# hits-mbm-dev/grappa

Hardware: AMD Instinct MI355X
Metric: molecules/sec (train step, energy+force loss) (higher is better)
Workload: dtype f32

## Files before the change

grappa_amd/_lib.py:

```python
import ctypes as C
import os

from . import settings

_HERE = os.path.dirname(os.path.abspath(__file__))
LIB_PATH = settings.read("LIB_PATH") or os.path.join(_HERE, "libgrappa_hip.so")

ABI_VERSION = 11
GEMM_GROUP4_MAX = 4
GEMM_GROUP_MAX = 16
GEMM_PRECISIONS = {"f32": 0, "f32_bf16x9": 1, "f32_bf16x6": 2, "bf16x3": 3, "bf16": 4, "f32_f16x3": 5}

c_float_p = C.POINTER(C.c_float)
c_int_p = C.POINTER(C.c_int)


class GemmDesc(C.Structure):
    _fields_ = [("M", C.c_int), ("N", C.c_int), ("K", C.c_int), ("a_kcontig", C.c_int), ("b_kcontig", C.c_int),
                ("A", C.c_void_p), ("lda", C.c_int), ("B", C.c_void_p), ("ldb", C.c_int), ("C", C.c_void_p), ("ldc", C.c_int),
                ("C2", C.c_void_p), ("ldc2", C.c_int), ("bias", C.c_void_p), ("res", C.c_void_p), ("ldres", C.c_int),
                ("aux", C.c_void_p), ("ldaux", C.c_int), ("pre", C.c_void_p), ("ldpre", C.c_int), ("a_colsum", C.c_void_p), ("act", C.c_int), ("drop_p", C.c_float), ("drop_seed", C.c_uint64),
                ("accumulate", C.c_int), ("precision", C.c_int),
                ("a_planes", C.c_int), ("b_planes", C.c_int), ("a_plane_stride", C.c_size_t), ("b_plane_stride", C.c_size_t),
                ("Cp", C.c_void_p), ("ldcp", C.c_int), ("cp_plane_stride", C.c_size_t),
                ("resp", C.c_void_p), ("ldresp", C.c_int), ("resp_plane_stride", C.c_size_t),
                ("auxp", C.c_void_p), ("ldauxp", C.c_int), ("auxp_plane_stride", C.c_size_t),
                ("cp_nplanes", C.c_int), ("resp_nplanes", C.c_int), ("auxp_nplanes", C.c_int), ("C1p", C.c_void_p), ("ldc1p", C.c_int),
                ("a_amax", C.c_void_p), ("b_amax", C.c_void_p), ("amax_bcast", C.c_int), ("out_amax", C.c_void_p),
                ("res_ln_mean", C.c_void_p), ("res_ln_rstd", C.c_void_p), ("res_ln_gamma", C.c_void_p), ("res_ln_beta", C.c_void_p),
                ("a_rowmax", C.c_void_p), ("b_rowmax", C.c_void_p),
                ("out_amax_parts", C.c_void_p), ("a_amax_nseg", C.c_int),
                ("plan_cfg", C.c_int), ("plan_nsplit", C.c_int), ("plan_tail", C.c_int), ("splitk_reduce", C.c_int), ("drop_salt", C.c_void_p)]


class LnFwdItem(C.Structure):
    _fields_ = [("M", C.c_int), ("W", C.c_int), ("x", C.c_void_p), ("ldx", C.c_int), ("gamma", C.c_void_p), ("beta", C.c_void_p), ("y", C.c_void_p),
                ("ldy", C.c_int), ("mean", C.c_void_p), ("rstd", C.c_void_p), ("y_amax", C.c_void_p)]


class LnBwdItem(C.Structure):
    _fields_ = [("M", C.c_int), ("W", C.c_int), ("dy", C.c_void_p), ("lddy", C.c_int), ("x", C.c_void_p), ("ldx", C.c_int), ("mean", C.c_void_p),
                ("rstd", C.c_void_p), ("gamma", C.c_void_p), ("dx", C.c_void_p), ("lddx", C.c_int), ("part", C.c_void_p), ("dx_amax", C.c_void_p)]


class ActDropoutItem(C.Structure):
    _fields_ = [("M", C.c_int), ("N", C.c_int), ("dy", C.c_void_p), ("lddy", C.c_int), ("y", C.c_void_p), ("ldy", C.c_int), ("drop_p", C.c_float),
                ("drop_seed", C.c_uint64), ("dz", C.c_void_p), ("lddz", C.c_int), ("dz_amax", C.c_void_p), ("drop_salt", C.c_void_p)]
# ... 97 lines not shown
    "grappa_split_planes_f32": (_i, [_vp, _i, _i, _vp, _i, _vp, _i, _sz, _i]),
    "grappa_split_pairs_f32": (_i, [_vp, _i, _i, _vp, _i, _vp, _vp, _i, _i]),
    "grappa_split_pairs_f32_batched": (_i, [_vp, _i, _i, _vp]),
    "grappa_amax_f32_workspace_bytes": (_sz, [_i, _i]),
    "grappa_amax_f32": (_i, [_vp, _i, _i, _vp, _i, _vp, _vp, _vp, _sz]),
    "grappa_amax_f32_batched": (_i, [_vp, _i, _vp]),
    "grappa_amax_reduce": (_i, [_vp, _i, C.POINTER(C.c_void_p), C.POINTER(C.c_int), _vp]),
    "grappa_amax_combine": (_i, [_vp, _i, _i, _vp, _vp]),
    "grappa_gemm_f32_workspace_bytes": (_sz, [_i, _i, _i]),
    "grappa_gemm_f32_plan": (_i, [_i, _i, _i, _i, c_int_p, c_int_p, c_int_p, c_int_p, c_int_p]),
    "grappa_gemm_f32_plan_desc": (_i, [C.POINTER(GemmDesc), c_int_p, c_int_p, c_int_p, c_int_p, c_int_p]),
    "grappa_gemm_f32_workspace_bytes_desc": (_sz, [C.POINTER(GemmDesc)]),
    "grappa_gemm_f32": (_i, [_vp, C.POINTER(GemmDesc), _vp, _sz]),
    "grappa_gemm_f32_grouped_workspace_bytes": (_sz, [C.POINTER(GemmDesc), _i]),
    "grappa_gemm_f32_grouped": (_i, [_vp, C.POINTER(GemmDesc), _i, _vp, _sz]),
    "grappa_gemm_f32_group_workspace_bytes": (_sz, [C.POINTER(GemmDesc), _i]),
    "grappa_gemm_f32_group": (_i, [_vp, C.POINTER(GemmDesc), _i, _vp, _sz]),
    "grappa_colsum_workspace_bytes": (_sz, [_i, _i]),
    "grappa_colsum_f32": (_i, [_vp, _i, _i, _vp, _i, _vp, _i, _vp, _sz]),
    "grappa_act_dropout_bwd_f32": (_i, [_vp, _i, _i, _vp, _i, _vp, _i, _f, _u64, _vp, _i, _vp]),
    "grappa_act_dropout_bwd_amax_f32": (_i, [_vp, _i, _i, _vp, _i, _vp, _i, _f, _u64, _vp, _i, _vp, _vp]),
    "grappa_layernorm_fwd_batched_f32": (_i, [_vp, C.POINTER(LnFwdItem), _i]),
    "grappa_layernorm_bwd_batched_f32": (_i, [_vp, C.POINTER(LnBwdItem), _i]),
    "grappa_act_dropout_bwd_batched_f32": (_i, [_vp, C.POINTER(ActDropoutItem), _i]),
    "grappa_seqattn_fwd_batched_f32": (_i, [_vp, C.POINTER(SeqAttnItem), _i]),
    "grappa_seqattn_bwd_batched_f32": (_i, [_vp, C.POINTER(SeqAttnItem), _i]),
    "grappa_act_dropout_bwd_pairs_f32": (_i, [_vp, _i, _i, _vp, _i, _vp, _i, _f, _u64, _vp, _i, _vp, _vp, _i, _vp]),
    "grappa_add_f32": (_i, [_vp, _sz, _vp, _vp, _vp]),
    "grappa_layernorm_fwd_f32": (_i, [_vp, _i, _i, _vp, _i, _vp, _vp, _vp, _i, _vp, _vp]),
    "grappa_layernorm_fwd_pairs_f32": (_i, [_vp, _i, _i, _vp, _i, _vp, _vp, _vp, _i, _vp, _vp, _vp, _vp, _i]),
# ... 134 lines not shown
```

grappa_amd/csrc/gemm_bf16x.hip:

```cpp
#include "gemm_common.h"

using namespace grappa_gemm;

#define GRAPPA_DECL(NAME)                                                                   \
    int grappa_bf16x_launch_##NAME(hipStream_t st, GemmParams& p, bool vec_kcontig);        \
    int grappa_bf16x_launch_group4_##NAME(hipStream_t st, const GemmGroup4& g, bool b_kcontig); \
    int grappa_bf16x_launch_grouped_##NAME(hipStream_t st, const GemmParams* d_ps, const int* d_wg_begin, int nprob, int total_wgs, bool vec, int psrc)
GRAPPA_DECL(x9);
GRAPPA_DECL(x6);
GRAPPA_DECL(x3);
GRAPPA_DECL(x1);
GRAPPA_DECL(h3);
#undef GRAPPA_DECL

int grappa_launch_gemm_bf16x_grouped(hipStream_t st, const GemmParams* d_ps, const int* d_wg_begin, int nprob, int total_wgs, int precision, bool vec, int psrc) {
    switch (precision) {
        case GRAPPA_GEMM_F32_BF16X9: return grappa_bf16x_launch_grouped_x9(st, d_ps, d_wg_begin, nprob, total_wgs, vec, psrc);
        case GRAPPA_GEMM_F32_BF16X6: return grappa_bf16x_launch_grouped_x6(st, d_ps, d_wg_begin, nprob, total_wgs, vec, psrc);
        case GRAPPA_GEMM_BF16X3: return grappa_bf16x_launch_grouped_x3(st, d_ps, d_wg_begin, nprob, total_wgs, vec, psrc);
        case GRAPPA_GEMM_BF16: return grappa_bf16x_launch_grouped_x1(st, d_ps, d_wg_begin, nprob, total_wgs, vec, psrc);
        case GRAPPA_GEMM_F32_F16X3: return grappa_bf16x_launch_grouped_h3(st, d_ps, d_wg_begin, nprob, total_wgs, vec, psrc);
        default: return GRAPPA_ERR_ARG;
    }
}

int grappa_launch_gemm_bf16x(hipStream_t st, GemmParams& p, int precision, bool vec_kcontig) {
    switch (precision) {
        case GRAPPA_GEMM_F32_BF16X9: return grappa_bf16x_launch_x9(st, p, vec_kcontig);
        case GRAPPA_GEMM_F32_BF16X6: return grappa_bf16x_launch_x6(st, p, vec_kcontig);
        case GRAPPA_GEMM_BF16X3: return grappa_bf16x_launch_x3(st, p, vec_kcontig);
        case GRAPPA_GEMM_BF16: return grappa_bf16x_launch_x1(st, p, vec_kcontig);
        case GRAPPA_GEMM_F32_F16X3: return grappa_bf16x_launch_h3(st, p, vec_kcontig);
        default: return GRAPPA_ERR_ARG;
    }
}

// ... 12 lines not shown
```

grappa_amd/csrc/gemm_bf16x_impl.h:

```cpp
#include "gemm_common.h"

using namespace grappa_gemm;

#ifndef GB_KNOCK
#define GB_KNOCK 0
#endif
#ifndef GB_STAGGER
#define GB_STAGGER 0
#endif

typedef __bf16 bf16x8 __attribute__((ext_vector_type(8)));
typedef __bf16 bf16x2 __attribute__((ext_vector_type(2)));
typedef _Float16 f16x8 __attribute__((ext_vector_type(8)));
typedef _Float16 f16x2 __attribute__((ext_vector_type(2)));

namespace {

constexpr int SK = 16;
constexpr int ROWB = 48;
#ifndef GB_AHEAD
#define GB_AHEAD 4
#endif
constexpr int AHEAD = GB_AHEAD;

// ... 327 lines not shown
    }
    __builtin_amdgcn_sched_barrier(0);
    if (!(GB_KNOCK == 5 && !TAIL)) __syncthreads();
    __builtin_amdgcn_sched_barrier(0);
    if (do_store && !(GB_KNOCK == 4 && !TAIL)) read_frags<NP, BM, BN, TM, TN, AV, BV>(nxt, wm0, wn0, lane, fn);
    if (GB_KNOCK == 4 && !TAIL) fn = fc;
    mfma_range<MODE, TM, TN, NFIRST, NM>(fc, acc);
    if (!TAIL) {
        __builtin_amdgcn_sched_group_barrier(0x002, 4, 0);
        ReadOrder<0, NM - NFIRST, (TM + TN) * NP + (AV ? TM * NP : 0) + (BV ? TN * NP : 0)>::emit();
    }
    __builtin_amdgcn_sched_barrier(0);
}

template <int NT, int MODE, int BM, int BN, int WN, bool AK, bool BKC, bool VEC, bool KMV, int PSRC = 0>
__device__ __forceinline__ void gemm_bf16x_body(const GemmParams& p, int nwg, int wgid) {
    static_assert(PSRC == 0 || (MODE == H3 && KMV && !AK && !BKC), "pair-format sources: the wgrad layout of the fp16-split arithmetic only");
    static_assert(PSRC >= 0 && PSRC <= 3, "PSRC 4 (formats per product) is resolved by the grouped kernel");
    constexpr bool pa_ = (PSRC & 1) != 0, pb_ = (PSRC & 2) != 0;
    constexpr int NP = Pieces<MODE>::NP, TM = 2, TN = BN / WN / 32;
    constexpr int NQA = BM * 4 / NT, NQB = BN * 4 / NT;
    constexpr bool AV = !AK && KMV, BV = !BKC && KMV;
    constexpr int PA = PieceBytes<BM, AV>::value;
    static_assert((NT / 64 / WN) * 64 == BM, "wavefront grid must cover the tile");
    extern __shared__ char smem[];
    const grappa_gemm_desc& d = p.d;
    if (GB_STAGGER > 0 && wgid < 256) {
        const int ph = (wgid >> 3) & 3;
        for (int i = 0; i < ph; ++i) __builtin_amdgcn_s_sleep(GB_STAGGER);
    }
    const TileCoord tc = map_logical(p, nwg, wgid);
    const int split = tc.split, tile_local = tc.tile_local, tile_n = tc.tile_n;
    const int m0 = tc.tile_m * BM, n0 = tile_n * BN;
    const int wave = threadIdx.x >> 6, lane = threadIdx.x & 63;
    const int wm0 = (wave / WN) * 64, wn0 = (wave % WN) * (BN / WN);
    const int lr = lane & 31, lh = lane >> 5;
    KRange kr;
    kr.kbeg = split * p.k_per_split;
    kr.kend = min(d.K, kr.kbeg + p.k_per_split);
    kr.nsteps = (kr.kend - kr.kbeg + SK - 1) / SK;
    const int nsteps = kr.nsteps;

    f32x16 acc[TM][TN];
#pragma unroll
    for (int i = 0; i < TM; ++i)
#pragma unroll
// ... 119 lines not shown
                for (int e = 0; e < 16; ++e) t += acc[i][j][e];
        if (t == 123.456f) p.d.C[0] = t;
        return;
    }
    tile_epilogue_rows<BM, BN, TM, TN>(p, acc, reinterpret_cast<float*>(smem + wave * EPI_WAVE_BYTES), m0, n0, wm0, wn0, lane, split, tile_local,
                                       p.vec_io != 0);
    if (p.nsplit > 1 && p.tickets) splitk_finish_tile<NT>(p, tile_local, reinterpret_cast<volatile int*>(smem));
}

template <int NT, int MODE, int BM, int BN, int WN, bool AK, bool BKC, bool VEC, bool KMV>
__global__ __launch_bounds__(NT, 2) void gemm_bf16x_kernel(GemmParams p) {
    gemm_bf16x_body<NT, MODE, BM, BN, WN, AK, BKC, VEC, KMV>(p, gridDim.x, blockIdx.x);
}

template <int NT, int MODE, int BM, int BN, int WN, bool AK, bool BKC, bool VEC, bool KMV, int PSRC = 0>
__global__ __launch_bounds__(NT, 2) void gemm_bf16x_grouped_kernel(const GemmParams* __restrict__ ps, const int* __restrict__ wg_begin, int nprob) {
    const int wg = blockIdx.x;
    int g = 0;
    while (g + 1 < nprob && wg >= wg_begin[g + 1]) ++g;
    if constexpr (PSRC == 4) {
        const int f = (ps[g].d.a_planes ? 1 : 0) | (ps[g].d.b_planes ? 2 : 0);
        const int nwg = wg_begin[g + 1] - wg_begin[g], id = wg - wg_begin[g];
        if (f == 0) gemm_bf16x_body<NT, MODE, BM, BN, WN, AK, BKC, VEC, KMV, 0>(ps[g], nwg, id);
        else if (f == 1) gemm_bf16x_body<NT, MODE, BM, BN, WN, AK, BKC, VEC, KMV, 1>(ps[g], nwg, id);
        else if (f == 2) gemm_bf16x_body<NT, MODE, BM, BN, WN, AK, BKC, VEC, KMV, 2>(ps[g], nwg, id);
        else gemm_bf16x_body<NT, MODE, BM, BN, WN, AK, BKC, VEC, KMV, 3>(ps[g], nwg, id);
    } else {
        gemm_bf16x_body<NT, MODE, BM, BN, WN, AK, BKC, VEC, KMV, PSRC>(ps[g], wg_begin[g + 1] - wg_begin[g], wg - wg_begin[g]);
    }
}

template <int NT, int MODE, int BM, int BN, int WN, bool AK, bool BKC, bool VEC, bool KMV>
__global__ __launch_bounds__(NT, 2) void gemm_bf16x_group4_kernel(GemmGroup4 g) {
    const int i = group4_find(g, blockIdx.x);
    gemm_bf16x_body<NT, MODE, BM, BN, WN, AK, BKC, VEC, KMV>(g.p[i], g.wg_begin[i + 1] - g.wg_begin[i], blockIdx.x - g.wg_begin[i]);
}

template <int NT, int MODE, int BM, int BN, int WN, bool AK, bool BKC, bool VEC, bool KMV>
int launch_group4_mode(hipStream_t st, const GemmGroup4& g) {
    constexpr size_t stages = 2 * (size_t)Pieces<MODE>::NP * (PieceBytes<BM, !AK && KMV>::value + PieceBytes<BN, !BKC && KMV>::value);
    constexpr size_t staging = (NT / 64) * (size_t)EPI_WAVE_BYTES;
    constexpr size_t smem = stages > staging ? stages : staging;
    auto kern = gemm_bf16x_group4_kernel<NT, MODE, BM, BN, WN, AK, BKC, VEC, KMV>;
// ... 27 lines not shown
int launch_layout(hipStream_t st, GemmParams& p, bool vec) {
    const grappa_gemm_desc& d = p.d;
    if (d.a_kcontig && d.b_kcontig) return vec ? launch_mode<NT, MODE, BM, BN, WN, true, true, true, false>(st, p) : launch_mode<NT, MODE, BM, BN, WN, true, true, false, false>(st, p);
    if (d.a_kcontig) return vec ? launch_mode<NT, MODE, BM, BN, WN, true, false, true, true>(st, p) : launch_mode<NT, MODE, BM, BN, WN, true, false, false, false>(st, p);
    return vec ? launch_mode<NT, MODE, BM, BN, WN, false, false, false, true>(st, p) : launch_mode<NT, MODE, BM, BN, WN, false, false, false, false>(st, p);
}

template <int MODE>
int launch_tile(hipStream_t st, GemmParams& p, bool vec) {
    if (p.bm == 256 && p.bn == 128) return launch_layout<512, MODE, 256, 128, 2>(st, p, vec);
    if (p.bm == 128 && p.bn == 128) return launch_layout<512, MODE, 128, 128, 4>(st, p, vec);
    return GRAPPA_ERR_ARG;
}

template <int MODE, bool KMV, int PSRC = 0>
int launch_grouped_wgrad(hipStream_t st, const GemmParams* d_ps, const int* d_wg_begin, int nprob, int total_wgs) {
    constexpr int NT = 512, BM = 256, BN = 128;
    constexpr size_t stages = 2 * (size_t)Pieces<MODE>::NP * (PieceBytes<BM, KMV>::value + PieceBytes<BN, KMV>::value);
    constexpr size_t staging = (NT / 64) * (size_t)EPI_WAVE_BYTES;
    constexpr size_t smem = stages > staging ? stages : staging;
    auto kern = gemm_bf16x_grouped_kernel<NT, MODE, BM, BN, 2, false, false, false, KMV, PSRC>;
    static bool attr_set = false;
    if (!attr_set) {
        if (hipFuncSetAttribute(reinterpret_cast<const void*>(kern), hipFuncAttributeMaxDynamicSharedMemorySize, (int)smem) != hipSuccess)
            return GRAPPA_ERR_LAUNCH;
        attr_set = true;
    }
    GRAPPA_LAUNCH(kern, dim3(total_wgs), dim3(NT), smem, st, d_ps, d_wg_begin, nprob);
    return grappa_launch_status();
}

}

template <int MODE>
int launch_group4(hipStream_t st, const GemmGroup4& g, bool b_kcontig) {
    if (b_kcontig) return launch_group4_mode<512, MODE, 256, 128, 2, true, true, true, false>(st, g);
    return launch_group4_mode<512, MODE, 256, 128, 2, true, false, true, true>(st, g);
}

#define GRAPPA_BF16X_MODE_FUNCS(MODE, NAME)                                                                                                  \
    int grappa_bf16x_launch_##NAME(hipStream_t st, GemmParams& p, bool vec_kcontig) { return launch_tile<MODE>(st, p, vec_kcontig); }       \
    int grappa_bf16x_launch_group4_##NAME(hipStream_t st, const GemmGroup4& g, bool b_kcontig) { return launch_group4<MODE>(st, g, b_kcontig); } \
    int grappa_bf16x_launch_grouped_##NAME(hipStream_t st, const GemmParams* d_ps, const int* d_wg_begin, int nprob, int total_wgs, bool vec, \
                                           int psrc) {                                                                                     \
        if constexpr (MODE == H3) {                                                                                                        \
            if (psrc != 0 && !vec) return GRAPPA_ERR_ARG;                                                                                  \
            if (psrc == 1) return launch_grouped_wgrad<MODE, true, 1>(st, d_ps, d_wg_begin, nprob, total_wgs);                             \
            if (psrc == 2) return launch_grouped_wgrad<MODE, true, 2>(st, d_ps, d_wg_begin, nprob, total_wgs);                             \
            if (psrc == 3) return launch_grouped_wgrad<MODE, true, 3>(st, d_ps, d_wg_begin, nprob, total_wgs);                             \
            if (psrc == 4) return launch_grouped_wgrad<MODE, true, 4>(st, d_ps, d_wg_begin, nprob, total_wgs);                             \
        } else if (psrc != 0) {                                                                                                            \
            return GRAPPA_ERR_ARG;                                                                                                         \
        }                                                                                                                                  \
        return vec ? launch_grouped_wgrad<MODE, true>(st, d_ps, d_wg_begin, nprob, total_wgs)                                              \
                   : launch_grouped_wgrad<MODE, false>(st, d_ps, d_wg_begin, nprob, total_wgs);                                            \
    }
```

grappa_amd/csrc/gemm_common.h:

```cpp
#pragma once
#include "common.h"

#ifndef GRAPPA_EPI_RES_LN
#define GRAPPA_EPI_RES_LN 1
#endif

typedef float f32x16 __attribute__((ext_vector_type(16)));

#ifndef GB_KNOCK
#define GB_KNOCK 0
#endif
namespace grappa_gemm {

constexpr int GEMM_BK = 32;

struct GemmParams {
    grappa_gemm_desc d;
    int k_per_split;
    int nsplit;
    float* slab;
    float* cs_slab;
    float drop_scale;
    int tiles_m, tiles_n;
    int tile_begin;
// ... 118 lines not shown
struct TileCoord {
    int split, tile_local, tile_m, tile_n;
};
__device__ inline TileCoord map_logical(const GemmParams& p, int nwg, int orig) {
    const int xcd = orig & 7, q = nwg >> 3, r = nwg & 7;
    const int wgid = (xcd < r ? xcd * (q + 1) : r * (q + 1) + (xcd - r) * q) + (orig >> 3);
    TileCoord t;
    t.split = wgid / p.ntiles_launch;
    t.tile_local = wgid - t.split * p.ntiles_launch;
    const int tile = p.tile_begin + t.tile_local;
    t.tile_m = tile / p.tiles_n;
    t.tile_n = tile % p.tiles_n;
    return t;
}
__device__ inline TileCoord map_workgroup(const GemmParams& p) { return map_logical(p, gridDim.x, blockIdx.x); }

template <int BM, int BN, int TM, int TN>
__device__ inline void tile_epilogue(const GemmParams& p, const f32x16 (&acc)[TM][TN], int m0, int n0, int wm0, int wn0, int lr, int lh,
                                     int split, int tile_local) {
    const grappa_gemm_desc& d = p.d;
    int ncol[TN];
    float bcol[TN];
#pragma unroll
    for (int j = 0; j < TN; ++j) {
        ncol[j] = n0 + wn0 + j * 32 + lr;
        bcol[j] = (d.bias && ncol[j] < d.N) ? d.bias[ncol[j]] : 0.0f;
    }
#pragma unroll
    for (int i = 0; i < TM; ++i)
#pragma unroll
// ... 361 lines not shown
```

grappa_amd/csrc/gemm_f32.hip:

```cpp
#include <cstdlib>
#include "gemm_common.h"

using namespace grappa_gemm;

int grappa_launch_gemm_bf16x(hipStream_t st, GemmParams& p, int precision, bool vec_kcontig);
int grappa_launch_gemm_planes(hipStream_t st, GemmParams& p, int precision);
int grappa_launch_gemm_pairs(hipStream_t st, GemmParams& p);
int grappa_launch_amax_combine(hipStream_t st, int M, int nseg, const unsigned* part, unsigned* out);
int grappa_launch_gemm_bf16x_group4(hipStream_t st, const GemmGroup4& g, int precision, bool b_kcontig);
int grappa_launch_gemm_pairs_group4(hipStream_t st, const GemmGroup4& g);
int grappa_launch_amax_combine4(hipStream_t st, int count, const int* M, const int* nseg, const unsigned* const* part, unsigned* const* out);
int grappa_launch_gemm_bf16x_grouped(hipStream_t st, const GemmParams* d_ps, const int* d_wg_begin, int nprob, int total_wgs, int precision, bool vec, int psrc);

namespace {

constexpr int BK = GEMM_BK;
constexpr int NTHREADS = 256;


template <int BROW, bool KCONT>
struct Tile {
    static constexpr int SIZE = KCONT ? BROW * (BK + 1) : BK * BROW;
    static constexpr int NV = BROW * BK / 4 / NTHREADS;
};

template <int BROW, bool KCONT>
__device__ inline void load_tile_vec(const float* __restrict__ src, int ld, int row0, int k0, int R, int Kend,
// ... 496 lines not shown
}

namespace {
constexpr int GROUP_MAX = GRAPPA_GEMM_GROUP_MAX;
struct GroupUpload {
    GemmParams p[8];
};
struct GroupIndex {
    int wg_begin[GROUP_MAX + 1], blk_begin[GROUP_MAX + 1];
};
__global__ void group_upload_kernel(GroupUpload u, int n, GemmParams* dst) {
    const int words = (int)(sizeof(GemmParams) / 4);
    for (int i = threadIdx.x; i < n * words; i += blockDim.x)
        reinterpret_cast<unsigned*>(dst)[i] = reinterpret_cast<const unsigned*>(u.p)[i];
}
__global__ void group_index_kernel(GroupIndex ix, int n, int* dst_wg, int* dst_blk, int* tickets, int ntickets) {
    for (int i = threadIdx.x; i <= n; i += blockDim.x) {
        dst_wg[i] = ix.wg_begin[i];
        dst_blk[i] = ix.blk_begin[i];
    }
    for (int i = threadIdx.x; i < ntickets; i += blockDim.x) tickets[i] = 0;
}

struct GroupPlan {
    int kps;
    int nsplit[GROUP_MAX], tiles[GROUP_MAX];
    int total_wgs;
    size_t slab_floats[GROUP_MAX], cs_floats[GROUP_MAX];
    size_t header_bytes, ticket_offset, total_bytes;
    int total_tickets;
};

bool pair_operand_ok(const void* q, int ld, int rows, const uint32_t* rowmax, int precision, int bcast_bit, int amax_bcast) {
    return precision == GRAPPA_GEMM_F32_F16X3 && rowmax != nullptr && (amax_bcast & bcast_bit) != 0 && (reinterpret_cast<uintptr_t>(q) & 15) == 0 &&
           (ld & 7) == 0 && (rows & 31) == 0 && ld >= 2 * rows;
// ... 37 lines not shown
        const double cost = (double)((wgs + 255) / 256) * 32768.0 * (kps + 160.0) / 307.0 + slab;
        if (cost < best) {
            best = cost;
            g.kps = kps;
        }
    }
    g.total_wgs = 0;
    size_t off = 0;
    for (int i = 0; i < n; ++i) {
        g.nsplit[i] = (descs[i].K + g.kps - 1) / g.kps;
        g.total_wgs += g.tiles[i] * g.nsplit[i];
        g.slab_floats[i] = g.nsplit[i] > 1 ? (size_t)g.nsplit[i] * g.tiles[i] * 256 * 128 : 0;
        g.cs_floats[i] = g.nsplit[i] > 1 ? (size_t)g.nsplit[i] * descs[i].M : 0;
        off += g.slab_floats[i] + g.cs_floats[i];
    }
    g.header_bytes = ((size_t)n * sizeof(GemmParams) + 2 * (GROUP_MAX + 1) * sizeof(int) + 255) / 256 * 256;
    g.ticket_offset = g.header_bytes + off * sizeof(float);
    g.total_tickets = 0;
    for (int i = 0; i < n; ++i) g.total_tickets += g.nsplit[i] > 1 ? g.tiles[i] : 0;
    g.total_bytes = g.ticket_offset + (size_t)g.total_tickets * sizeof(int);
    return g;
}
}

extern "C" size_t grappa_gemm_f32_grouped_workspace_bytes(const grappa_gemm_desc* descs, int n) {
    if (!descs || n <= 0 || n > GROUP_MAX) return 0;
    return plan_group(descs, n).total_bytes;
}

extern "C" int grappa_gemm_f32_grouped(void* stream, const grappa_gemm_desc* descs, int n, void* ws, size_t ws_bytes) {
    if (!descs || n <= 0 || n > GROUP_MAX) return GRAPPA_ERR_ARG;
    const int precision = descs[0].precision;
    int psrc = (descs[0].a_planes ? 1 : 0) | (descs[0].b_planes ? 2 : 0);
    for (int i = 0; i < n; ++i) {
        if (!group_desc_ok(descs[i], precision)) return GRAPPA_ERR_ARG;
        if (((descs[i].a_planes ? 1 : 0) | (descs[i].b_planes ? 2 : 0)) != psrc) psrc = 4;
    }
    const GroupPlan g = plan_group(descs, n);
    if (!ws || ws_bytes < g.total_bytes) return GRAPPA_ERR_WORKSPACE;
    hipStream_t st = reinterpret_cast<hipStream_t>(stream);
    GemmParams* d_ps = reinterpret_cast<GemmParams*>(ws);
    int* d_wg = reinterpret_cast<int*>(reinterpret_cast<char*>(ws) + (size_t)n * sizeof(GemmParams));
    int* d_blk = d_wg + (GROUP_MAX + 1);
    float* slab = reinterpret_cast<float*>(reinterpret_cast<char*>(ws) + g.header_bytes);
    GroupIndex ix;
    GroupUpload up;
    ix.wg_begin[0] = ix.blk_begin[0] = 0;
    const bool in_kernel = splitk_in_kernel(descs[0]);
    int* tickets = reinterpret_cast<int*>(reinterpret_cast<char*>(ws) + g.ticket_offset);
    int* next_ticket = tickets;
    auto al16 = [](const void* q, int ld) { return q == nullptr || ((reinterpret_cast<uintptr_t>(q) & 15) == 0 && (ld & 3) == 0); };
    int total_blocks = 0;
    bool vec = true;
    for (int i = 0; i < n; ++i) {
        const grappa_gemm_desc& d = descs[i];
        vec = vec && (reinterpret_cast<uintptr_t>(d.A) & 15) == 0 && (d.lda & 3) == 0 && ((d.M + 3) & ~3) <= d.lda &&
              (reinterpret_cast<uintptr_t>(d.B) & 15) == 0 && (d.ldb & 3) == 0 && ((d.N + 3) & ~3) <= d.ldb;
    }
// ... 26 lines not shown
            p.vec_io = al16(d.C, d.ldc) && al16(d.C2, d.ldc2) && al16(d.pre, d.ldpre) && al16(d.res, d.ldres) && al16(d.aux, d.ldaux);
            p.amax_part = nullptr;
            p.amax_seg = 32;
            p.epi_class = 0;
            ix.wg_begin[i + 1] = ix.wg_begin[i] + g.tiles[i] * g.nsplit[i];
            int blocks = 0;
            if (p.nsplit > 1 && !in_kernel) {
                blocks = (int)(((size_t)g.tiles[i] * 256 * 128 / 4 + REDUCE_THREADS - 1) / REDUCE_THREADS);
                if (blocks > 1024) blocks = 1024;
            }
            ix.blk_begin[i + 1] = ix.blk_begin[i] + blocks;
            total_blocks = ix.blk_begin[i + 1];
        }
        GRAPPA_LAUNCH(group_upload_kernel, dim3(1), dim3(256), 0, st, up, cnt, d_ps + i0);
    }
    GRAPPA_LAUNCH(group_index_kernel, dim3(1), dim3(256), 0, st, ix, n, d_wg, d_blk, tickets, in_kernel ? g.total_tickets : 0);
    if (grappa_launch_status() != GRAPPA_OK) return GRAPPA_ERR_LAUNCH;
    int rc = grappa_launch_gemm_bf16x_grouped(st, d_ps, d_wg, n, g.total_wgs, precision, vec, psrc);
    if (rc != GRAPPA_OK) return rc;
    if (total_blocks > 0) {
        GRAPPA_LAUNCH(gemm_splitk_reduce_grouped_kernel, dim3(total_blocks), dim3(REDUCE_THREADS), 0, st, d_ps, d_blk, n);
        rc = grappa_launch_status();
    }
    return rc;
}

extern "C" int grappa_gemm_f32(void* stream, const grappa_gemm_desc* d, void* ws, size_t ws_bytes) {
    if (!d || !d->A || !d->B || (!d->C && !d->Cp && !d->C1p)) return GRAPPA_ERR_ARG;
    if (!d->C && (d->C2 || d->accumulate)) return GRAPPA_ERR_ARG;
    if (d->C1p && (d->C || d->C2) ) return GRAPPA_ERR_ARG;
    if (d->C1p && !d->Cp) return GRAPPA_ERR_ARG;
    for (int np : {d->cp_nplanes, d->resp_nplanes, d->auxp_nplanes})
        if (np != 0 && np != 1 && np != 3) return GRAPPA_ERR_ARG;
// ... 220 lines not shown
```

include/grappa_hip.h:

```cpp
#ifndef GRAPPA_HIP_H
#define GRAPPA_HIP_H

#include <stddef.h>
#include <stdint.h>

#ifdef __cplusplus
extern "C" {
#endif

#define GRAPPA_OK 0
#define GRAPPA_ERR_ARG (-1)
#define GRAPPA_ERR_LAUNCH (-2)
#define GRAPPA_ERR_WORKSPACE (-3)

#define GRAPPA_ABI_VERSION 11
int grappa_abi_version(void);
const char* grappa_build_arch(void);
long long grappa_launch_count(int reset);

#define GRAPPA_ACT_NONE 0
#define GRAPPA_ACT_ELU 1

#define GRAPPA_GEMM_F32_MFMA 0
#define GRAPPA_GEMM_F32_BF16X9 1
// ... 19 lines not shown
    uint64_t drop_seed;
    int accumulate;
    int precision;
    int a_planes, b_planes;
    size_t a_plane_stride, b_plane_stride;
    uint16_t* Cp; int ldcp; size_t cp_plane_stride;
    const uint16_t* resp; int ldresp; size_t resp_plane_stride;
    const uint16_t* auxp; int ldauxp; size_t auxp_plane_stride;
    int cp_nplanes, resp_nplanes, auxp_nplanes;
    uint16_t* C1p; int ldc1p;
    const uint32_t* a_amax; const uint32_t* b_amax; int amax_bcast;
    uint32_t* out_amax;
    const float* res_ln_mean; const float* res_ln_rstd; const float* res_ln_gamma; const float* res_ln_beta;
    const uint32_t* a_rowmax; const uint32_t* b_rowmax;
    uint32_t* out_amax_parts; int a_amax_nseg;
    int plan_cfg, plan_nsplit, plan_tail, splitk_reduce;
    const uint64_t* drop_salt;
} grappa_gemm_desc;

size_t grappa_amax_f32_workspace_bytes(int R, int C);
int grappa_amax_f32(void* stream, int R, int C, const float* x, int ldx, uint32_t* row_amax, uint32_t* col_amax, void* ws, size_t ws_bytes);
typedef struct grappa_amax_item {
    const float* x; int R, C, ld, pad_;
    uint32_t* row_amax; uint32_t* col_amax;
} grappa_amax_item;
int grappa_amax_f32_batched(void* stream, int count, const grappa_amax_item* descs);
int grappa_amax_reduce(void* stream, int count, const uint32_t* const* in, const int* n, uint32_t* out);
int grappa_amax_combine(void* stream, int M, int nseg, const uint32_t* parts, uint32_t* out);

int grappa_split_planes_f32(void* stream, int R, int C, const float* x, int ldx, uint16_t* planes, int ldp, size_t plane_stride,
                            int transpose);
// ... 2 lines not shown
typedef struct grappa_split_pairs_item {
    const float* x; const uint32_t* amax; uint16_t* pairs;
    int R, C, ldx, ldp, transpose, tile_begin;
} grappa_split_pairs_item;
int grappa_split_pairs_f32_batched(void* stream, int count, int total_tiles, const grappa_split_pairs_item* items);

size_t grappa_gemm_f32_workspace_bytes(int M, int N, int K);
size_t grappa_gemm_f32_workspace_bytes_desc(const grappa_gemm_desc* d);
int grappa_gemm_f32_plan(int M, int N, int K, int precision, int* tile_m, int* tile_n, int* nsplit, int* tail_tiles, int* tail_nsplit);
int grappa_gemm_f32_plan_desc(const grappa_gemm_desc* d, int* tile_m, int* tile_n, int* nsplit, int* tail_tiles, int* tail_nsplit);
int grappa_gemm_f32(void* stream, const grappa_gemm_desc* d, void* ws, size_t ws_bytes);

#define GRAPPA_GEMM_GROUP_MAX 16
size_t grappa_gemm_f32_grouped_workspace_bytes(const grappa_gemm_desc* descs, int n);
int grappa_gemm_f32_grouped(void* stream, const grappa_gemm_desc* descs, int n, void* ws, size_t ws_bytes);
size_t grappa_gemm_f32_group_workspace_bytes(const grappa_gemm_desc* descs, int n);
int grappa_gemm_f32_group(void* stream, const grappa_gemm_desc* descs, int n, void* ws, size_t ws_bytes);

size_t grappa_colsum_workspace_bytes(int M, int N);
int grappa_colsum_f32(void* stream, int M, int N, const float* x, int ldx, float* out, int accumulate,
                      void* ws, size_t ws_bytes);

int grappa_act_dropout_bwd_f32(void* stream, int M, int N, const float* dy, int lddy, const float* y, int ldy,
                               float drop_p, uint64_t drop_seed, float* dz, int lddz, const uint64_t* drop_salt);
int grappa_act_dropout_bwd_amax_f32(void* stream, int M, int N, const float* dy, int lddy, const float* y, int ldy,
                                    float drop_p, uint64_t drop_seed, float* dz, int lddz, uint32_t* dz_amax, const uint64_t* drop_salt);
#define GRAPPA_ROW_BATCH_MAX 4
typedef struct grappa_ln_fwd_item {
    int M, W; const float* x; int ldx; const float* gamma; const float* beta; float* y; int ldy; float* mean; float* rstd; uint32_t* y_amax;
} grappa_ln_fwd_item;
// ... 340 lines not shown
```

Measured before the change: 7735.

## Deal grouped wgrad GEMM split-K slices across eight queues by cost

Adds a host-side scheduler that breaks each grouped wgrad GEMM problem into per-split slices, sorts them by cost (tiles times K range), and greedily assigns them to eight queues interleaved by workgroup id (wg&7). The assignment packs slices into 32-tile chunks and is uploaded as a GroupSlices table. The grouped kernel then maps each workgroup straight to (problem, split, tile) instead of walking wg_begin in linear order. The goal is to balance long and short K slices across XCD-like queues and cut tail imbalance. In exchange it enlarges the workspace header, may launch padding workgroups that exit early, and adds host work on every call.

Result: no change. 7768, median of 6 (+0.4%).

```diff
diff --git a/grappa_amd/_lib.py b/grappa_amd/_lib.py
--- a/grappa_amd/_lib.py
+++ b/grappa_amd/_lib.py
@@ -30,7 +30,9 @@
                 ("res_ln_mean", C.c_void_p), ("res_ln_rstd", C.c_void_p), ("res_ln_gamma", C.c_void_p), ("res_ln_beta", C.c_void_p),
                 ("a_rowmax", C.c_void_p), ("b_rowmax", C.c_void_p),
                 ("out_amax_parts", C.c_void_p), ("a_amax_nseg", C.c_int),
-                ("plan_cfg", C.c_int), ("plan_nsplit", C.c_int), ("plan_tail", C.c_int), ("splitk_reduce", C.c_int), ("drop_salt", C.c_void_p)]
+                ("plan_cfg", C.c_int), ("plan_nsplit", C.c_int), ("plan_tail", C.c_int), ("splitk_reduce", C.c_int),
+                ("wgrad_order", C.c_int),
+                ("drop_salt", C.c_void_p)]
 
 
 class LnFwdItem(C.Structure):
@@ -158,6 +160,7 @@
     "grappa_gemm_f32": (_i, [_vp, C.POINTER(GemmDesc), _vp, _sz]),
     "grappa_gemm_f32_grouped_workspace_bytes": (_sz, [C.POINTER(GemmDesc), _i]),
     "grappa_gemm_f32_grouped": (_i, [_vp, C.POINTER(GemmDesc), _i, _vp, _sz]),
+    "grappa_gemm_f32_grouped_order": (_i, [C.POINTER(GemmDesc), _i, c_int_p, _i]),
     "grappa_gemm_f32_group_workspace_bytes": (_sz, [C.POINTER(GemmDesc), _i]),
     "grappa_gemm_f32_group": (_i, [_vp, C.POINTER(GemmDesc), _i, _vp, _sz]),
     "grappa_colsum_workspace_bytes": (_sz, [_i, _i]),
diff --git a/grappa_amd/csrc/gemm_bf16x.hip b/grappa_amd/csrc/gemm_bf16x.hip
--- a/grappa_amd/csrc/gemm_bf16x.hip
+++ b/grappa_amd/csrc/gemm_bf16x.hip
@@ -5,7 +5,7 @@
 #define GRAPPA_DECL(NAME)                                                                   \
     int grappa_bf16x_launch_##NAME(hipStream_t st, GemmParams& p, bool vec_kcontig);        \
     int grappa_bf16x_launch_group4_##NAME(hipStream_t st, const GemmGroup4& g, bool b_kcontig); \
-    int grappa_bf16x_launch_grouped_##NAME(hipStream_t st, const GemmParams* d_ps, const int* d_wg_begin, int nprob, int total_wgs, bool vec, int psrc)
+    int grappa_bf16x_launch_grouped_##NAME(hipStream_t st, const GemmParams* d_ps, const int* d_wg_begin, int nprob, int total_wgs, bool vec, int psrc, const GroupSlices* d_slices)
 GRAPPA_DECL(x9);
 GRAPPA_DECL(x6);
 GRAPPA_DECL(x3);
@@ -13,13 +13,13 @@
 GRAPPA_DECL(h3);
 #undef GRAPPA_DECL
 
-int grappa_launch_gemm_bf16x_grouped(hipStream_t st, const GemmParams* d_ps, const int* d_wg_begin, int nprob, int total_wgs, int precision, bool vec, int psrc) {
+int grappa_launch_gemm_bf16x_grouped(hipStream_t st, const GemmParams* d_ps, const int* d_wg_begin, int nprob, int total_wgs, int precision, bool vec, int psrc, const GroupSlices* d_slices) {
     switch (precision) {
-        case GRAPPA_GEMM_F32_BF16X9: return grappa_bf16x_launch_grouped_x9(st, d_ps, d_wg_begin, nprob, total_wgs, vec, psrc);
-        case GRAPPA_GEMM_F32_BF16X6: return grappa_bf16x_launch_grouped_x6(st, d_ps, d_wg_begin, nprob, total_wgs, vec, psrc);
-        case GRAPPA_GEMM_BF16X3: return grappa_bf16x_launch_grouped_x3(st, d_ps, d_wg_begin, nprob, total_wgs, vec, psrc);
-        case GRAPPA_GEMM_BF16: return grappa_bf16x_launch_grouped_x1(st, d_ps, d_wg_begin, nprob, total_wgs, vec, psrc);
-        case GRAPPA_GEMM_F32_F16X3: return grappa_bf16x_launch_grouped_h3(st, d_ps, d_wg_begin, nprob, total_wgs, vec, psrc);
+        case GRAPPA_GEMM_F32_BF16X9: return grappa_bf16x_launch_grouped_x9(st, d_ps, d_wg_begin, nprob, total_wgs, vec, psrc, d_slices);
+        case GRAPPA_GEMM_F32_BF16X6: return grappa_bf16x_launch_grouped_x6(st, d_ps, d_wg_begin, nprob, total_wgs, vec, psrc, d_slices);
+        case GRAPPA_GEMM_BF16X3: return grappa_bf16x_launch_grouped_x3(st, d_ps, d_wg_begin, nprob, total_wgs, vec, psrc, d_slices);
+        case GRAPPA_GEMM_BF16: return grappa_bf16x_launch_grouped_x1(st, d_ps, d_wg_begin, nprob, total_wgs, vec, psrc, d_slices);
+        case GRAPPA_GEMM_F32_F16X3: return grappa_bf16x_launch_grouped_h3(st, d_ps, d_wg_begin, nprob, total_wgs, vec, psrc, d_slices);
         default: return GRAPPA_ERR_ARG;
     }
 }
diff --git a/grappa_amd/csrc/gemm_bf16x_impl.h b/grappa_amd/csrc/gemm_bf16x_impl.h
--- a/grappa_amd/csrc/gemm_bf16x_impl.h
+++ b/grappa_amd/csrc/gemm_bf16x_impl.h
@@ -365,7 +365,7 @@
 }
 
 template <int NT, int MODE, int BM, int BN, int WN, bool AK, bool BKC, bool VEC, bool KMV, int PSRC = 0>
-__device__ __forceinline__ void gemm_bf16x_body(const GemmParams& p, int nwg, int wgid) {
+__device__ __forceinline__ void gemm_bf16x_body(const GemmParams& p, int nwg, int wgid, const TileCoord* given = nullptr) {
     static_assert(PSRC == 0 || (MODE == H3 && KMV && !AK && !BKC), "pair-format sources: the wgrad layout of the fp16-split arithmetic only");
     static_assert(PSRC >= 0 && PSRC <= 3, "PSRC 4 (formats per product) is resolved by the grouped kernel");
     constexpr bool pa_ = (PSRC & 1) != 0, pb_ = (PSRC & 2) != 0;
@@ -380,7 +380,7 @@
         const int ph = (wgid >> 3) & 3;
         for (int i = 0; i < ph; ++i) __builtin_amdgcn_s_sleep(GB_STAGGER);
     }
-    const TileCoord tc = map_logical(p, nwg, wgid);
+    const TileCoord tc = given ? *given : map_logical(p, nwg, wgid);
     const int split = tc.split, tile_local = tc.tile_local, tile_n = tc.tile_n;
     const int m0 = tc.tile_m * BM, n0 = tile_n * BN;
     const int wave = threadIdx.x >> 6, lane = threadIdx.x & 63;
@@ -530,19 +530,34 @@
 }
 
 template <int NT, int MODE, int BM, int BN, int WN, bool AK, bool BKC, bool VEC, bool KMV, int PSRC = 0>
-__global__ __launch_bounds__(NT, 2) void gemm_bf16x_grouped_kernel(const GemmParams* __restrict__ ps, const int* __restrict__ wg_begin, int nprob) {
+__global__ __launch_bounds__(NT, 2) void gemm_bf16x_grouped_kernel(const GemmParams* __restrict__ ps, const int* __restrict__ wg_begin, int nprob,
+                                                                   const GroupSlices* __restrict__ slices) {
     const int wg = blockIdx.x;
-    int g = 0;
-    while (g + 1 < nprob && wg >= wg_begin[g + 1]) ++g;
+    int g = 0, nwg = 0, id = 0;
+    TileCoord tc;
+    if (slices) {
+        const int q = wg & 7, e = wg >> 3;
+        if (e >= slices->qend[q]) return;
+        int i = slices->qbeg[q];
+        const int last = slices->qbeg[q + 1] - 1;
+        while (i < last && e >= slices->tile0[i + 1]) ++i;
+        const int sl = slices->slice[i];
+        g = sl & 15;
+        tc = map_given(ps[g], sl >> 4, e - slices->tile0[i]);
+    } else {
+        while (g + 1 < nprob && wg >= wg_begin[g + 1]) ++g;
+        nwg = wg_begin[g + 1] - wg_begin[g];
+        id = wg - wg_begin[g];
+        tc = map_logical(ps[g], nwg, id);
+    }
     if constexpr (PSRC == 4) {
         const int f = (ps[g].d.a_planes ? 1 : 0) | (ps[g].d.b_planes ? 2 : 0);
-        const int nwg = wg_begin[g + 1] - wg_begin[g], id = wg - wg_begin[g];
-        if (f == 0) gemm_bf16x_body<NT, MODE, BM, BN, WN, AK, BKC, VEC, KMV, 0>(ps[g], nwg, id);
-        else if (f == 1) gemm_bf16x_body<NT, MODE, BM, BN, WN, AK, BKC, VEC, KMV, 1>(ps[g], nwg, id);
-        else if (f == 2) gemm_bf16x_body<NT, MODE, BM, BN, WN, AK, BKC, VEC, KMV, 2>(ps[g], nwg, id);
-        else gemm_bf16x_body<NT, MODE, BM, BN, WN, AK, BKC, VEC, KMV, 3>(ps[g], nwg, id);
+        if (f == 0) gemm_bf16x_body<NT, MODE, BM, BN, WN, AK, BKC, VEC, KMV, 0>(ps[g], nwg, id, &tc);
+        else if (f == 1) gemm_bf16x_body<NT, MODE, BM, BN, WN, AK, BKC, VEC, KMV, 1>(ps[g], nwg, id, &tc);
+        else if (f == 2) gemm_bf16x_body<NT, MODE, BM, BN, WN, AK, BKC, VEC, KMV, 2>(ps[g], nwg, id, &tc);
+        else gemm_bf16x_body<NT, MODE, BM, BN, WN, AK, BKC, VEC, KMV, 3>(ps[g], nwg, id, &tc);
     } else {
-        gemm_bf16x_body<NT, MODE, BM, BN, WN, AK, BKC, VEC, KMV, PSRC>(ps[g], wg_begin[g + 1] - wg_begin[g], wg - wg_begin[g]);
+        gemm_bf16x_body<NT, MODE, BM, BN, WN, AK, BKC, VEC, KMV, PSRC>(ps[g], nwg, id, &tc);
     }
 }
 
@@ -600,7 +615,7 @@
 }
 
 template <int MODE, bool KMV, int PSRC = 0>
-int launch_grouped_wgrad(hipStream_t st, const GemmParams* d_ps, const int* d_wg_begin, int nprob, int total_wgs) {
+int launch_grouped_wgrad(hipStream_t st, const GemmParams* d_ps, const int* d_wg_begin, int nprob, int total_wgs, const GroupSlices* d_slices) {
     constexpr int NT = 512, BM = 256, BN = 128;
     constexpr size_t stages = 2 * (size_t)Pieces<MODE>::NP * (PieceBytes<BM, KMV>::value + PieceBytes<BN, KMV>::value);
     constexpr size_t staging = (NT / 64) * (size_t)EPI_WAVE_BYTES;
@@ -612,7 +627,7 @@
             return GRAPPA_ERR_LAUNCH;
         attr_set = true;
     }
-    GRAPPA_LAUNCH(kern, dim3(total_wgs), dim3(NT), smem, st, d_ps, d_wg_begin, nprob);
+    GRAPPA_LAUNCH(kern, dim3(total_wgs), dim3(NT), smem, st, d_ps, d_wg_begin, nprob, d_slices);
     return grappa_launch_status();
 }
 
@@ -628,16 +643,16 @@
     int grappa_bf16x_launch_##NAME(hipStream_t st, GemmParams& p, bool vec_kcontig) { return launch_tile<MODE>(st, p, vec_kcontig); }       \
     int grappa_bf16x_launch_group4_##NAME(hipStream_t st, const GemmGroup4& g, bool b_kcontig) { return launch_group4<MODE>(st, g, b_kcontig); } \
     int grappa_bf16x_launch_grouped_##NAME(hipStream_t st, const GemmParams* d_ps, const int* d_wg_begin, int nprob, int total_wgs, bool vec, \
-                                           int psrc) {                                                                                     \
+                                           int psrc, const GroupSlices* d_slices) {                                                                                     \
         if constexpr (MODE == H3) {                                                                                                        \
             if (psrc != 0 && !vec) return GRAPPA_ERR_ARG;                                                                                  \
-            if (psrc == 1) return launch_grouped_wgrad<MODE, true, 1>(st, d_ps, d_wg_begin, nprob, total_wgs);                             \
-            if (psrc == 2) return launch_grouped_wgrad<MODE, true, 2>(st, d_ps, d_wg_begin, nprob, total_wgs);                             \
-            if (psrc == 3) return launch_grouped_wgrad<MODE, true, 3>(st, d_ps, d_wg_begin, nprob, total_wgs);                             \
-            if (psrc == 4) return launch_grouped_wgrad<MODE, true, 4>(st, d_ps, d_wg_begin, nprob, total_wgs);                             \
+            if (psrc == 1) return launch_grouped_wgrad<MODE, true, 1>(st, d_ps, d_wg_begin, nprob, total_wgs, d_slices);                             \
+            if (psrc == 2) return launch_grouped_wgrad<MODE, true, 2>(st, d_ps, d_wg_begin, nprob, total_wgs, d_slices);                             \
+            if (psrc == 3) return launch_grouped_wgrad<MODE, true, 3>(st, d_ps, d_wg_begin, nprob, total_wgs, d_slices);                             \
+            if (psrc == 4) return launch_grouped_wgrad<MODE, true, 4>(st, d_ps, d_wg_begin, nprob, total_wgs, d_slices);                             \
         } else if (psrc != 0) {                                                                                                            \
             return GRAPPA_ERR_ARG;                                                                                                         \
         }                                                                                                                                  \
-        return vec ? launch_grouped_wgrad<MODE, true>(st, d_ps, d_wg_begin, nprob, total_wgs)                                              \
-                   : launch_grouped_wgrad<MODE, false>(st, d_ps, d_wg_begin, nprob, total_wgs);                                            \
-    }
+        return vec ? launch_grouped_wgrad<MODE, true>(st, d_ps, d_wg_begin, nprob, total_wgs, d_slices)                                              \
+                   : launch_grouped_wgrad<MODE, false>(st, d_ps, d_wg_begin, nprob, total_wgs, d_slices);                                            \
+    }
diff --git a/grappa_amd/csrc/gemm_common.h b/grappa_amd/csrc/gemm_common.h
--- a/grappa_amd/csrc/gemm_common.h
+++ b/grappa_amd/csrc/gemm_common.h
@@ -156,6 +156,22 @@
     return t;
 }
 __device__ inline TileCoord map_workgroup(const GemmParams& p) { return map_logical(p, gridDim.x, blockIdx.x); }
+__device__ inline TileCoord map_given(const GemmParams& p, int split, int tile_local) {
+    TileCoord t;
+    t.split = split;
+    t.tile_local = tile_local;
+    const int tile = p.tile_begin + tile_local;
+    t.tile_m = tile / p.tiles_n;
+    t.tile_n = tile % p.tiles_n;
+    return t;
+}
+
+constexpr int GROUP_SLICES_MAX = 512;
+struct GroupSlices {
+    int qbeg[9], qend[8];
+    int tile0[GROUP_SLICES_MAX];
+    uint16_t slice[GROUP_SLICES_MAX];
+};
 
 template <int BM, int BN, int TM, int TN>
 __device__ inline void tile_epilogue(const GemmParams& p, const f32x16 (&acc)[TM][TN], int m0, int n0, int wm0, int wn0, int lr, int lh,
diff --git a/grappa_amd/csrc/gemm_f32.hip b/grappa_amd/csrc/gemm_f32.hip
--- a/grappa_amd/csrc/gemm_f32.hip
+++ b/grappa_amd/csrc/gemm_f32.hip
@@ -10,7 +10,7 @@
 int grappa_launch_gemm_bf16x_group4(hipStream_t st, const GemmGroup4& g, int precision, bool b_kcontig);
 int grappa_launch_gemm_pairs_group4(hipStream_t st, const GemmGroup4& g);
 int grappa_launch_amax_combine4(hipStream_t st, int count, const int* M, const int* nseg, const unsigned* const* part, unsigned* const* out);
-int grappa_launch_gemm_bf16x_grouped(hipStream_t st, const GemmParams* d_ps, const int* d_wg_begin, int nprob, int total_wgs, int precision, bool vec, int psrc);
+int grappa_launch_gemm_bf16x_grouped(hipStream_t st, const GemmParams* d_ps, const int* d_wg_begin, int nprob, int total_wgs, int precision, bool vec, int psrc, const GroupSlices* d_slices);
 
 namespace {
 
@@ -537,11 +537,15 @@
     for (int i = threadIdx.x; i < n * words; i += blockDim.x)
         reinterpret_cast<unsigned*>(dst)[i] = reinterpret_cast<const unsigned*>(u.p)[i];
 }
-__global__ void group_index_kernel(GroupIndex ix, int n, int* dst_wg, int* dst_blk, int* tickets, int ntickets) {
+__global__ void group_index_kernel(GroupIndex ix, GroupSlices sl, int n, int* dst_wg, int* dst_blk, GroupSlices* dst_sl, int* tickets, int ntickets) {
     for (int i = threadIdx.x; i <= n; i += blockDim.x) {
         dst_wg[i] = ix.wg_begin[i];
         dst_blk[i] = ix.blk_begin[i];
     }
+    static_assert(sizeof(GroupSlices) % 4 == 0, "copied by words");
+    if (dst_sl)
+        for (int i = threadIdx.x; i < (int)(sizeof(GroupSlices) / 4); i += blockDim.x)
+            reinterpret_cast<unsigned*>(dst_sl)[i] = reinterpret_cast<const unsigned*>(&sl)[i];
     for (int i = threadIdx.x; i < ntickets; i += blockDim.x) tickets[i] = 0;
 }
 
@@ -609,18 +613,94 @@
         g.cs_floats[i] = g.nsplit[i] > 1 ? (size_t)g.nsplit[i] * descs[i].M : 0;
         off += g.slab_floats[i] + g.cs_floats[i];
     }
-    g.header_bytes = ((size_t)n * sizeof(GemmParams) + 2 * (GROUP_MAX + 1) * sizeof(int) + 255) / 256 * 256;
+    g.header_bytes = ((size_t)n * sizeof(GemmParams) + 2 * (GROUP_MAX + 1) * sizeof(int) + sizeof(GroupSlices) + 255) / 256 * 256;
     g.ticket_offset = g.header_bytes + off * sizeof(float);
     g.total_tickets = 0;
     for (int i = 0; i < n; ++i) g.total_tickets += g.nsplit[i] > 1 ? g.tiles[i] : 0;
     g.total_bytes = g.ticket_offset + (size_t)g.total_tickets * sizeof(int);
     return g;
 }
+
+int deal_slices(const GroupPlan& g, const grappa_gemm_desc* descs, int n, GroupSlices& t) {
+    struct Slice { int prob, split, tiles; long cost; };
+    Slice sl[GROUP_SLICES_MAX];
+    int order[GROUP_SLICES_MAX], ns = 0;
+    for (int i = 0; i < n; ++i)
+        for (int s = 0; s < g.nsplit[i]; ++s) {
+            if (ns == GROUP_SLICES_MAX || s >= 4096) return 0;
+            const int kend = descs[i].K < (s + 1) * g.kps ? descs[i].K : (s + 1) * g.kps;
+            sl[ns] = {i, s, g.tiles[i], (long)g.tiles[i] * (kend - s * g.kps)};
+            order[ns] = ns;
+            ++ns;
+        }
+    for (int a = 1; a < ns; ++a) {
+        const int v = order[a];
+        int b = a;
+        for (; b > 0 && sl[order[b - 1]].cost < sl[v].cost; --b) order[b] = order[b - 1];
+        order[b] = v;
+    }
+    const int cap = (g.total_wgs + 8 * 31) / 8;
+    long load[8] = {0, 0, 0, 0, 0, 0, 0, 0};
+    int len[8] = {0, 0, 0, 0, 0, 0, 0, 0}, cnt[8] = {0, 0, 0, 0, 0, 0, 0, 0};
+    int member[8][GROUP_SLICES_MAX];
+    for (int a = 0; a < ns; ++a) {
+        const Slice& s = sl[order[a]];
+        int q = -1, any = 0;
+        for (int c = 0; c < 8; ++c) {
+            if (load[c] < load[any]) any = c;
+            if (len[c] + s.tiles <= cap && (q < 0 || load[c] < load[q])) q = c;
+        }
+        if (q < 0) q = any;
+        member[q][cnt[q]++] = order[a];
+        load[q] += s.cost;
+        len[q] += s.tiles;
+    }
+    int at = 0, longest = 0;
+    for (int q = 0; q < 8; ++q) {
+        t.qbeg[q] = at;
+        int pos = 0;
+        for (int left = cnt[q]; left > 0; --left) {
+            const int room = 32 - pos % 32;
+            int pick = 0;
+            if (room < 32)
+                for (int c = 0; c < left; ++c)
+                    if (sl[member[q][c]].tiles <= room) { pick = c; break; }
+            const Slice& s = sl[member[q][pick]];
+            t.slice[at] = (uint16_t)(s.prob | (s.split << 4));
+            t.tile0[at] = pos;
+            pos += s.tiles;
+            ++at;
+            for (int c = pick; c + 1 < left; ++c) member[q][c] = member[q][c + 1];
+        }
+        t.qend[q] = pos;
+        longest = pos > longest ? pos : longest;
+    }
+    t.qbeg[8] = at;
+    for (int i = at; i < GROUP_SLICES_MAX; ++i) { t.slice[i] = 0; t.tile0[i] = 0; }
+    return 8 * longest;
+}
 }
 
 extern "C" size_t grappa_gemm_f32_grouped_workspace_bytes(const grappa_gemm_desc* descs, int n) {
     if (!descs || n <= 0 || n > GROUP_MAX) return 0;
     return plan_group(descs, n).total_bytes;
+}
+
+extern "C" int grappa_gemm_f32_grouped_order(const grappa_gemm_desc* descs, int n, int* wg, int cap) {
+    if (!descs || n <= 0 || n > GROUP_MAX || (cap > 0 && !wg)) return GRAPPA_ERR_ARG;
+    GroupSlices t;
+    const int grid = descs[0].wgrad_order == 0 ? deal_slices(plan_group(descs, n), descs, n, t) : 0;
+    for (int b = 0; b < grid && b < cap; ++b) {
+        const int q = b & 7, e = b >> 3;
+        wg[3 * b] = wg[3 * b + 1] = wg[3 * b + 2] = -1;
+        if (e >= t.qend[q]) continue;
+        int i = t.qbeg[q];
+        while (i < t.qbeg[q + 1] - 1 && e >= t.tile0[i + 1]) ++i;
+        wg[3 * b] = t.slice[i] & 15;
+        wg[3 * b + 1] = t.slice[i] >> 4;
+        wg[3 * b + 2] = e - t.tile0[i];
+    }
+    return grid;
 }
 
 extern "C" int grappa_gemm_f32_grouped(void* stream, const grappa_gemm_desc* descs, int n, void* ws, size_t ws_bytes) {
@@ -637,6 +717,7 @@
     GemmParams* d_ps = reinterpret_cast<GemmParams*>(ws);
     int* d_wg = reinterpret_cast<int*>(reinterpret_cast<char*>(ws) + (size_t)n * sizeof(GemmParams));
     int* d_blk = d_wg + (GROUP_MAX + 1);
+    GroupSlices* d_slices = reinterpret_cast<GroupSlices*>(d_blk + (GROUP_MAX + 1));
     float* slab = reinterpret_cast<float*>(reinterpret_cast<char*>(ws) + g.header_bytes);
     GroupIndex ix;
     GroupUpload up;
@@ -693,9 +774,15 @@
         }
         GRAPPA_LAUNCH(group_upload_kernel, dim3(1), dim3(256), 0, st, up, cnt, d_ps + i0);
     }
-    GRAPPA_LAUNCH(group_index_kernel, dim3(1), dim3(256), 0, st, ix, n, d_wg, d_blk, tickets, in_kernel ? g.total_tickets : 0);
+    GroupSlices sl;
+    const int sliced_grid = descs[0].wgrad_order == 0 ? deal_slices(g, descs, n, sl) : 0;
+    if (sliced_grid == 0) {
+        sl = GroupSlices{};
+        d_slices = nullptr;
+    }
+    GRAPPA_LAUNCH(group_index_kernel, dim3(1), dim3(256), 0, st, ix, sl, n, d_wg, d_blk, d_slices, tickets, in_kernel ? g.total_tickets : 0);
     if (grappa_launch_status() != GRAPPA_OK) return GRAPPA_ERR_LAUNCH;
-    int rc = grappa_launch_gemm_bf16x_grouped(st, d_ps, d_wg, n, g.total_wgs, precision, vec, psrc);
+    int rc = grappa_launch_gemm_bf16x_grouped(st, d_ps, d_wg, n, d_slices ? sliced_grid : g.total_wgs, precision, vec, psrc, d_slices);
     if (rc != GRAPPA_OK) return rc;
     if (total_blocks > 0) {
         GRAPPA_LAUNCH(gemm_splitk_reduce_grouped_kernel, dim3(total_blocks), dim3(REDUCE_THREADS), 0, st, d_ps, d_blk, n);
diff --git a/include/grappa_hip.h b/include/grappa_hip.h
--- a/include/grappa_hip.h
+++ b/include/grappa_hip.h
@@ -57,7 +57,7 @@
     const float* res_ln_mean; const float* res_ln_rstd; const float* res_ln_gamma; const float* res_ln_beta;
     const uint32_t* a_rowmax; const uint32_t* b_rowmax;
     uint32_t* out_amax_parts; int a_amax_nseg;
-    int plan_cfg, plan_nsplit, plan_tail, splitk_reduce;
+    int plan_cfg, plan_nsplit, plan_tail, splitk_reduce, wgrad_order;
     const uint64_t* drop_salt;
 } grappa_gemm_desc;
 
@@ -90,6 +90,7 @@
 #define GRAPPA_GEMM_GROUP_MAX 16
 size_t grappa_gemm_f32_grouped_workspace_bytes(const grappa_gemm_desc* descs, int n);
 int grappa_gemm_f32_grouped(void* stream, const grappa_gemm_desc* descs, int n, void* ws, size_t ws_bytes);
+int grappa_gemm_f32_grouped_order(const grappa_gemm_desc* descs, int n, int* wg, int cap);
 size_t grappa_gemm_f32_group_workspace_bytes(const grappa_gemm_desc* descs, int n);
 int grappa_gemm_f32_group(void* stream, const grappa_gemm_desc* descs, int n, void* ws, size_t ws_bytes);
 
```
